# zpelgrims/pota

Hardware: AMD Instinct MI355X
Metric: bidir redistribution Msamples/s at 4K, double-gauss 50mm (higher is better)
Workload: dtype f64

## Files before the change

pota_amd/csrc/lentil_hip.hip:

```cpp
#include <hip/hip_runtime.h>
#include <hip/hip_ext.h>

#include <algorithm>
#include <atomic>
#include <chrono>
#include <cmath>
#include <cstdio>
#include <cstdlib>
#include <cstring>
#include <deque>
#include <mutex>
#include <new>
#include <string>
#include <vector>

#include "lentil_kernels.h"
#include "lentil_closest_replay.h"
#include "lentil_tl_chroma_mgpu.h"
#include "lentil_lens_jit.h"
#include "lentil_camera_rays.h"
#include "lentil_trace_points.h"
#include "lentil_list_draws.h"
#include "generated/embedded_sources.inc"

// ... 191 lines not shown
  uint32_t last_scan_launches = 0;
  int32_t dirty_lo = 0, dirty_hi = 0;
  bool dirty_known = false;
  hipEvent_t scans_done = nullptr;
  uint32_t margin_low_rate = 10;
  uint32_t batch_margin16 = 4;
  uint32_t unknown_credit = 7;
  hipEvent_t ev_solve = nullptr, ev_slow1 = nullptr;
  hipStream_t aux_stream = nullptr;
  hipEvent_t ev_crypto = nullptr;
  bool crypto_direct_enqueued = false;
  bool streams_concurrent = false;
  hipStream_t slow1_stream = nullptr;
  hipEvent_t ev_slow = nullptr, ev_round = nullptr;
  bool early_resolve_pending = false;
  bool late_resolve_done = false;
  bool resolved_valid = false;
  hipEvent_t ev_acc1 = nullptr, ev_res = nullptr;
  hipStream_t pub_stream = nullptr;
  hipEvent_t pub_done = nullptr;
  bool pass_pending = false;
  bool closest_deferred = false;
  uint32_t visit_id_base = 0;
  DevCounters *d_ctr = nullptr;
  std::vector<DevCounters> h_ctr;
  DevCounters *h_ctr_pinned = nullptr;
  bool h_ctr_valid = false;
  lentil_draw_record *d_log = nullptr;
  uint64_t log_cap = 0;
  bool timed_draw = false, timed_resolve = false;
  hipEvent_t ev_scan_k[2] = {nullptr, nullptr};
  bool scan_kernel_timed = false;
  uint32_t xor_state[4] = {123456789u, 362436069u, 521288629u, 88675123u};
  uint32_t *d_xor = nullptr, *d_tlc_res = nullptr;
  uint64_t *d_tlc_off = nullptr;
  uint2 *d_tlc_tasks = nullptr;
  uint64_t tlc_res_cap = 0, tlc_off_cap = 0, tlc_tasks_cap = 0;
  uint4 *d_xor_jump = nullptr, *d_tlc_entry = nullptr;
  uint64_t *d_tlc_val = nullptr;
  uint64_t tlc_entry_cap = 0, tlc_val_cap = 0;
  std::vector<uint32_t> tlc_gids;
  bool tlc_have_entries = false, tlc_rewalk = false;
  uint32_t *d_tlc_bound = nullptr, *d_tlc_probed = nullptr, *d_tlc_occ = nullptr;
  uint64_t tlc_bound_cap = 0, tlc_probed_cap = 0, tlc_occ_cap = 0, tlc_occ_n = 0, tlc_occ_slots = 0;
  bool tlc_occ_valid = false, pass_rerun = false;
  uint64_t tlc_items = 0, tlc_dependent = 0, tlc_gathered = 0;
  double lens_housing_radius = 0.0;
  float4 *d_dummy = nullptr;
  float *d_cam_keys = nullptr;
  float shutter_t0 = 0.0f, shutter_inv_dt = 1.0f;
  uint32_t n_cam_keys = 0;
  bool async_end = true;
  bool clear_pending = false;
  hipEvent_t ev_pre_clear = nullptr, ev_clear = nullptr;
  int ready_blocks = 2;
  struct Slot {
    hipEvent_t ev[5] = {nullptr, nullptr, nullptr, nullptr, nullptr};
    hipEvent_t ev_scan_k[2] = {nullptr, nullptr};
    hipEvent_t ev_tail = nullptr;
    DevCounters *h_ctr_pinned = nullptr;
    bool timing_open = false;
    bool timed_draw = false, timed_resolve = false, scan_kernel_timed = false;
  } slots[3];
  int slot = 0;
  struct Inflight {
    int slot = 0;
    bool abandoned = false;
    bool resolve_requested = false;
    StreamTail t;
    VisitsDev V{};
    bool have_visits = false;
  };
  std::deque<Inflight> inflight;
  bool holds_turn = false;
  lentil_pass_totals totals{};
  std::vector<std::string> notes;
  lentil_probe_fn probe_fn = nullptr;
  void *probe_user = nullptr;
  bool probe_c2w_given = false;
  float probe_c2w[16];
  std::vector<float> h_cam_keys;
  float *d_c2w_keys = nullptr;
  bool c2w_keys_valid = false;
// ... 48 lines not shown
static std::mutex g_stall_notes_mutex;
static std::vector<std::string> g_stall_notes;

static int fail(lentil_hip_ctx *ctx, int code, const std::string &msg) {
  if (ctx) ctx->err = msg; else g_err = msg;
  return code;
}
#define HIP_TRY(ctx, call)                                                                   \
  do {                                                                                       \
    hipError_t e_ = (call);                                                                  \
    if (e_ != hipSuccess)                                                                    \
      return fail(ctx, LENTIL_ERR_HIP, std::string(#call) + ": " + hipGetErrorString(e_));   \
  } while (0)
static int settle(lentil_hip_ctx *ctx);
static int probe_round(lentil_hip_ctx *ctx, int ci, const DrawArgs &da, hipStream_t st);
static int join_clear(lentil_hip_ctx *ctx);
static void harvest_ready(lentil_hip_ctx *ctx);
static int resolve_range(lentil_hip_ctx *ctx, uint64_t p_begin, uint64_t p_end);
#define CHECK_CTX_PIPELINED(ctx) \
  if (!(ctx)) return fail(nullptr, LENTIL_ERR_INVALID, "null context")
#define CHECK_CTX(ctx)                                                     \
  do {                                                                     \
    if (!(ctx)) return fail(nullptr, LENTIL_ERR_INVALID, "null context"); \
    if (!(ctx)->inflight.empty()) {                                        \
      const int rc_settle_ = settle(ctx);                                  \
      if (rc_settle_) return rc_settle_;                                   \
    }                                                                      \
    if ((ctx)->clear_pending) {                                            \
      const int rc_join_ = join_clear(ctx);                                \
      if (rc_join_) return rc_join_;                                       \
    }                                                                      \
  } while (0)

static int join_clear(lentil_hip_ctx *ctx) {
  if (!ctx->clear_pending) return LENTIL_OK;
  HIP_TRY(ctx, hipSetDevice(ctx->device));
  HIP_TRY(ctx, hipStreamWaitEvent(ctx->stream, ctx->ev_clear, 0));
  ctx->clear_pending = false;
  return LENTIL_OK;
}

static inline void ht_mark(lentil_hip_ctx *ctx, const char *what) {
  if (!host_trace_passes()) return;
  if (ctx->trace.passes_left < 0) ctx->trace.passes_left = host_trace_passes();
  if (ctx->trace.passes_left == 0) return;
  ctx->trace.marks.emplace_back(what, (int64_t)std::chrono::duration_cast<std::chrono::nanoseconds>(
// ... 84 lines not shown
  return LENTIL_OK;
}

LENTIL_API int lentil_hip_create(int device, lentil_hip_ctx **out_ctx) {
  if (!out_ctx) return fail(nullptr, LENTIL_ERR_INVALID, "out_ctx is null");
  *out_ctx = nullptr;
  int count = 0;
  hipError_t e = hipGetDeviceCount(&count);
  if (e != hipSuccess || count <= 0)
    return fail(nullptr, LENTIL_ERR_HIP, std::string("no HIP device: ") + hipGetErrorString(e));
  if (device < 0 || device >= count) return fail(nullptr, LENTIL_ERR_INVALID, "device index out of range");
  lentil_hip_ctx *ctx = new (std::nothrow) lentil_hip_ctx();
  if (!ctx) return fail(nullptr, LENTIL_ERR_NOMEM, "out of host memory");
  ctx->device = device;
  HIP_TRY(ctx, hipSetDevice(device));
  hipDeviceProp_t prop;
  HIP_TRY(ctx, hipGetDeviceProperties(&prop, device));
  ctx->num_cu = prop.multiProcessorCount > 0 ? prop.multiProcessorCount : 256;
  HIP_TRY(ctx, hipStreamCreateWithFlags(&ctx->stream, hipStreamNonBlocking));
  for (auto &ev : ctx->ev) HIP_TRY(ctx, hipEventCreate(&ev));
  if (const char *nc = getenv("LENTIL_CHUNKS")) { ctx->n_chunks = atoi(nc); }
  if (ctx->n_chunks < 1) ctx->n_chunks = 1;
  if (ctx->n_chunks > 16) ctx->n_chunks = 16;
  HIP_TRY(ctx, hipMalloc(&ctx->d_ctr, sizeof(DevCounters) * (ctx->n_chunks + 1)));
  HIP_TRY(ctx, hipHostMalloc((void **)&ctx->h_ctr_pinned, sizeof(DevCounters) * ctx->n_chunks, hipHostMallocDefault));
  memset(ctx->h_ctr_pinned, 0, sizeof(DevCounters) * ctx->n_chunks);
  if (const char *e = getenv("LENTIL_ASYNC_END")) ctx->async_end = e[0] != '0';
  HIP_TRY(ctx, hipEventCreateWithFlags(&ctx->ev_pre_clear, hipEventDisableTiming));
  HIP_TRY(ctx, hipEventCreateWithFlags(&ctx->ev_clear, hipEventDisableTiming));
  if (const char *e = getenv("LENTIL_READY_ACCEPT_BLOCKS")) { ctx->ready_blocks = atoi(e); if (ctx->ready_blocks < 1) ctx->ready_blocks = 1; if (ctx->ready_blocks > 6) ctx->ready_blocks = 6; }
  HIP_TRY(ctx, hipEventCreate(&ctx->ev_scan_k[0]));
  HIP_TRY(ctx, hipEventCreate(&ctx->ev_scan_k[1]));
  for (int si = 0; si < 3; ++si) {
    lentil_hip_ctx::Slot &sl = ctx->slots[si];
    if (si == 0) {
      for (int i = 0; i < 5; ++i) sl.ev[i] = ctx->ev[i];
      sl.ev_scan_k[0] = ctx->ev_scan_k[0]; sl.ev_scan_k[1] = ctx->ev_scan_k[1];
      sl.h_ctr_pinned = ctx->h_ctr_pinned;
    } else {
      for (int i = 0; i < 5; ++i) HIP_TRY(ctx, hipEventCreate(&sl.ev[i]));
      HIP_TRY(ctx, hipEventCreate(&sl.ev_scan_k[0]));
      HIP_TRY(ctx, hipEventCreate(&sl.ev_scan_k[1]));
      HIP_TRY(ctx, hipHostMalloc((void **)&sl.h_ctr_pinned, sizeof(DevCounters) * ctx->n_chunks, hipHostMallocDefault));
      memset(sl.h_ctr_pinned, 0, sizeof(DevCounters) * ctx->n_chunks);
    }
    HIP_TRY(ctx, hipEventCreateWithFlags(&sl.ev_tail, hipEventDisableTiming));
  }
  HIP_TRY(ctx, hipMalloc(&ctx->d_dummy, 64 * sizeof(float4)));
  HIP_TRY(ctx, hipMemsetAsync(ctx->d_ctr, 0, sizeof(DevCounters) * (ctx->n_chunks + 1), ctx->stream));
  ctx->chunks.resize(ctx->n_chunks);
  for (auto &ch : ctx->chunks) {
    HIP_TRY(ctx, hipStreamCreateWithFlags(&ch.stream, hipStreamNonBlocking));
    HIP_TRY(ctx, hipEventCreateWithFlags(&ch.scanned, hipEventDisableTiming));
    HIP_TRY(ctx, hipEventCreateWithFlags(&ch.done, hipEventDisableTiming));
  }
  HIP_TRY(ctx, hipEventCreateWithFlags(&ctx->scans_done, hipEventDisableTiming));
  HIP_TRY(ctx, hipStreamCreateWithFlags(&ctx->pub_stream, hipStreamNonBlocking));
  HIP_TRY(ctx, hipEventCreateWithFlags(&ctx->ev_slow, hipEventDisableTiming));
  HIP_TRY(ctx, hipEventCreateWithFlags(&ctx->ev_round, hipEventDisableTiming));
  HIP_TRY(ctx, hipEventCreateWithFlags(&ctx->pub_done, hipEventDisableTiming));
  HIP_TRY(ctx, hipEventCreateWithFlags(&ctx->ev_acc1, hipEventDisableTiming));
  HIP_TRY(ctx, hipEventCreateWithFlags(&ctx->ev_res, hipEventDisableTiming));
  HIP_TRY(ctx, hipEventCreateWithFlags(&ctx->ev_solve, hipEventDisableTiming));
  HIP_TRY(ctx, hipEventCreateWithFlags(&ctx->ev_slow1, hipEventDisableTiming));
  HIP_TRY(ctx, hipStreamCreateWithFlags(&ctx->slow1_stream, hipStreamNonBlocking));
  HIP_TRY(ctx, hipEventCreateWithFlags(&ctx->ev_crypto, hipEventDisableTiming));
  { const int rc = pick_concurrent_streams(ctx); if (rc) return rc; }
  if (const char *e = getenv("LENTIL_INJECT_STALL")) ctx->inject_stall_at = atoi(e);
  if (const char *e = getenv("LENTIL_PROBE_DEVICE_CAP")) { const long long v = atoll(e); ctx->probe_dev_cap = v > 0 ? (uint64_t)v : 0; }
  if (const char *ft = getenv("LENTIL_FORCE_TABLES")) ctx->use_generated = !(ft[0] == '1');
  if (const char *fc = getenv("LENTIL_FIRST_CHUNK_FRAC")) {
    const double f = atof(fc);
// ... 132 lines not shown
    if (ch.stream) (void)hipStreamDestroy(ch.stream);
  }
  if (ctx->scans_done) (void)hipEventDestroy(ctx->scans_done);
  if (ctx->pub_stream) { (void)hipStreamSynchronize(ctx->pub_stream); (void)hipStreamDestroy(ctx->pub_stream); }
  if (ctx->pub_done) (void)hipEventDestroy(ctx->pub_done);
  if (ctx->ev_slow) (void)hipEventDestroy(ctx->ev_slow);
  if (ctx->ev_round) (void)hipEventDestroy(ctx->ev_round);
  if (ctx->ev_pre_clear) (void)hipEventDestroy(ctx->ev_pre_clear);
  if (ctx->ev_clear) (void)hipEventDestroy(ctx->ev_clear);
  for (lentil_hip_ctx::Slot &sl : ctx->slots) {
    for (hipEvent_t e : sl.ev) if (e) (void)hipEventDestroy(e);
    if (sl.ev_scan_k[0]) (void)hipEventDestroy(sl.ev_scan_k[0]);
    if (sl.ev_scan_k[1]) (void)hipEventDestroy(sl.ev_scan_k[1]);
    if (sl.ev_tail) (void)hipEventDestroy(sl.ev_tail);
    if (sl.h_ctr_pinned) (void)hipHostFree(sl.h_ctr_pinned);
  }
  if (ctx->ev_acc1) (void)hipEventDestroy(ctx->ev_acc1);
  if (ctx->ev_res) (void)hipEventDestroy(ctx->ev_res);
  if (ctx->ev_solve) (void)hipEventDestroy(ctx->ev_solve);
  if (ctx->ev_slow1) (void)hipEventDestroy(ctx->ev_slow1);
  if (ctx->slow1_stream) { (void)hipStreamSynchronize(ctx->slow1_stream); (void)hipStreamDestroy(ctx->slow1_stream); }
  if (ctx->aux_stream) { (void)hipStreamSynchronize(ctx->aux_stream); (void)hipStreamDestroy(ctx->aux_stream); }
  if (ctx->ev_crypto) (void)hipEventDestroy(ctx->ev_crypto);
  (void)hipFree(ctx->d_ctr);
  (void)hipFree(ctx->d_ranges);
  (void)hipFree(ctx->d_c2w_keys);
  probe_buf_free(ctx->tlc_pb);
  probe_buf_free(ctx->ld_pb);
  for (auto &ch : ctx->chunks) probe_buf_free(ch.pb);
  if (ctx->jit_module) (void)hipModuleUnload(ctx->jit_module);
  (void)hipFree(ctx->d_bm_land); (void)hipFree(ctx->d_bm_box); (void)hipFree(ctx->d_bm_npass);
  (void)hipFree(ctx->d_xor); (void)hipFree(ctx->d_tlc_res); (void)hipFree(ctx->d_tlc_off); (void)hipFree(ctx->d_tlc_tasks);
  (void)hipFree(ctx->d_xor_jump); (void)hipFree(ctx->d_tlc_entry); (void)hipFree(ctx->d_tlc_val);
  (void)hipFree(ctx->d_tlc_bound); (void)hipFree(ctx->d_tlc_probed); (void)hipFree(ctx->d_tlc_occ);
  (void)hipFree(ctx->d_log);
  if (ctx->stream) (void)hipStreamDestroy(ctx->stream);
  delete ctx;
  return LENTIL_OK;
}

LENTIL_API const char *lentil_hip_last_error(const lentil_hip_ctx *ctx) {
  return ctx ? ctx->err.c_str() : g_err.c_str();
}

LENTIL_API const char *lentil_hip_last_redo_note(const lentil_hip_ctx *ctx) {
  return ctx ? ctx->redo_note.c_str() : "";
}
// ... 803 lines not shown
  apply_camera_motion(ctx);
  ctx->V.id_base = ctx->visit_id_base;
  rc = ensure_worklist(ctx, v->n);
  if (rc) return rc;
  ctx->have_visits = true;
  ++ctx->visits_gen;
  return LENTIL_OK;
}

LENTIL_API int lentil_hip_clear_frame(lentil_hip_ctx *ctx) {
  CHECK_CTX_PIPELINED(ctx);
  if (!ctx->inflight.empty()) { ctx->inflight.back().abandoned = true; harvest_ready(ctx); }
  if (!ctx->trace.marks.empty()) { ht_mark(ctx, "next_clear"); ht_dump(ctx); }
  ht_mark(ctx, "clear{");
  ctx->resolved_valid = false;
  if (!ctx->have_frame) return fail(ctx, LENTIL_ERR_INVALID, "no frame allocated");
  HIP_TRY(ctx, hipSetDevice(ctx->device));
  if (ctx->F.touched) {
    const uint64_t n_groups = (ctx->F.np + 63) / 64;
    uint64_t blocks = (n_groups + 255) / 256;
    const uint64_t max_blocks = (uint64_t)ctx->num_cu * 4;
    if (blocks > max_blocks) blocks = max_blocks;
    hipStream_t cs = ctx->stream;
    const bool off = ctx->streams_concurrent && ctx->stream_mode && !ctx->chunks.empty() && ctx->chunks[0].stream && !ctx->clear_pending;
    if (off) {
      cs = ctx->chunks[0].stream;
      HIP_TRY(ctx, hipEventRecord(ctx->ev_pre_clear, ctx->stream));
      HIP_TRY(ctx, hipStreamWaitEvent(cs, ctx->ev_pre_clear, 0));
    }
    hipLaunchKernelGGL(clear_touched_kernel, dim3((unsigned)blocks), dim3(256), 0, cs, ctx->F, n_groups);
    HIP_TRY(ctx, hipGetLastError());
    if (off) {
      HIP_TRY(ctx, hipEventRecord(ctx->ev_clear, cs));
      ctx->clear_pending = true;
    }
    ctx->F.touched = nullptr;
    ctx->F.touched_px = nullptr;
  } else {
  { const int rcj = join_clear(ctx); if (rcj) return rcj; }
  uint64_t p0 = 0, p1 = ctx->F.np;
  if (ctx->dirty_known && !ctx->pass_pending) {
    p0 = (uint64_t)(ctx->dirty_lo < 0 ? 0 : ctx->dirty_lo) * ctx->P.xres;
    p1 = (uint64_t)(ctx->dirty_hi < ctx->dirty_lo ? ctx->dirty_lo : ctx->dirty_hi) * ctx->P.xres;
    if (p1 > ctx->F.np) p1 = ctx->F.np;
    if (p0 > p1) p0 = p1;
  }
  if (p1 > p0) {
    HIP_TRY(ctx, hipMemsetAsync(ctx->F.acc + p0 * ctx->F.stride, 0, (p1 - p0) * ctx->F.stride * sizeof(float), ctx->stream));
    if (ctx->F.zkey) HIP_TRY(ctx, hipMemsetAsync(ctx->F.zkey + p0, 0xFF, (p1 - p0) * sizeof(unsigned long long), ctx->stream));
    if (ctx->F.zkey_dbg) HIP_TRY(ctx, hipMemsetAsync(ctx->F.zkey_dbg + p0, 0xFF, (p1 - p0) * sizeof(unsigned long long), ctx->stream));
  }
  }
  { const int rc = crypto_clear(ctx); if (rc) return rc; }
  ctx->F.dir = nullptr;
  ctx->cleared_since_pass = true;
  ctx->dirty_lo = ctx->dirty_hi = 0;
  ctx->dirty_known = true;
  ctx->pass_pending = false;
  ht_mark(ctx, "}clear");
  return LENTIL_OK;
}

template <typename T>
static int grow(lentil_hip_ctx *ctx, T **p, uint64_t need) {
  (void)hipFree(*p);
  *p = nullptr;
  HIP_TRY(ctx, hipMalloc((void **)p, need * sizeof(T)));
  return LENTIL_OK;
}

template <bool kStream>
static void launch_solve_po(lentil_hip_ctx *ctx, const DrawArgs &da, hipStream_t st, unsigned blocks) {
  const bool chroma = da.n_channels == 3;
  bool launched = false;
#define LENTIL_LAUNCH_GEN(NAME)                                                                          \
// ... 873 lines not shown
    }
  T.scan_launches += ctx->last_scan_launches ? ctx->last_scan_launches : 1u;
  if ((uint64_t)ctx->last_rounds > T.rounds_max) T.rounds_max = (uint64_t)ctx->last_rounds;
}

static int harvest_front(lentil_hip_ctx *ctx) {
  lentil_hip_ctx::Inflight in = ctx->inflight.front();
  ctx->inflight.pop_front();
  lentil_hip_ctx::Slot &sl = ctx->slots[in.slot];
  int rc = LENTIL_OK;
  HIP_TRY(ctx, hipSetDevice(ctx->device));
  {
    const hipError_t e = hipEventSynchronize(sl.ev[2]);
    if (e != hipSuccess) { release_turn(ctx); return fail(ctx, LENTIL_ERR_HIP, std::string("waiting for a pass's end: ") + hipGetErrorString(e)); }
  }
  {
    float ms = 0.f;
    if (hipEventElapsedTime(&ms, sl.ev[0], sl.ev[2]) == hipSuccess) {
      const double m = (double)ms + 0.3;
      if (!in.t.calibrates_now && m > ctx->longest_pass_ms && m < 200.0) { ctx->longest_pass_ms = m; ctx->longest_pass_visits = in.V.n; ctx->longest_pass_sum = ctx->est_sum_total; }
    } else (void)hipGetLastError();
  }
  const bool can_fix = !in.abandoned;
  ctx->last_blind = 1; ctx->last_fallback = 0; ctx->last_rounds = 0; ctx->last_scan_launches = 1; ctx->last_streamed = 1;
  ctx->h_ctr_valid = false;
  std::swap(ctx->V, in.V);
  std::swap(ctx->have_visits, in.have_visits);
  bool streamed = true;
  ctx->stall_redo = false;
  rc = streamed_finish(ctx, in.t, sl.h_ctr_pinned, can_fix, &streamed);
  if (rc == LENTIL_OK && can_fix) {
    if (ctx->stall_redo) rc = redo_after_stall(ctx);
    if (rc == LENTIL_OK && in.t.did_more) {
      ctx->resolved_valid = false;
      ctx->early_resolve_pending = false;
      (void)hipEventRecord(sl.ev[2], ctx->stream);
    }
    if (rc == LENTIL_OK) rc = pass_finish(ctx);
    if (rc == LENTIL_OK && in.resolve_requested && !ctx->resolved_valid) rc = resolve_range(ctx, 0, ctx->F.np);
  }
  ctx->stall_redo = false;
  ++ctx->totals.deferred;
  if (in.abandoned) ++ctx->totals.abandoned;
  if (rc == LENTIL_OK) account_pass(ctx);
  std::swap(ctx->V, in.V);
  std::swap(ctx->have_visits, in.have_visits);
// ... 14 lines not shown
static void harvest_ready(lentil_hip_ctx *ctx) {
  while (!ctx->inflight.empty() && ctx->inflight.front().abandoned) {
    if (hipEventQuery(ctx->slots[ctx->inflight.front().slot].ev[2]) != hipSuccess) { (void)hipGetLastError(); return; }
    (void)harvest_front(ctx);
  }
}

static int begin_slot(lentil_hip_ctx *ctx) {
  lentil_hip_ctx::Slot &cur = ctx->slots[ctx->slot];
  cur.timed_draw = ctx->timed_draw; cur.timed_resolve = ctx->timed_resolve; cur.scan_kernel_timed = ctx->scan_kernel_timed;
  const int next = (ctx->slot + 1) % 3;
  while (ctx->inflight.size() >= 2 || (!ctx->inflight.empty() && ctx->inflight.front().slot == next)) {
    const int rc = harvest_front(ctx);
    if (rc) return rc;
  }
  flush_timing(ctx, ctx->slot, false);
  ctx->slot = -1;
  flush_timing(ctx, next, true);
  ctx->slot = next;
  lentil_hip_ctx::Slot &n = ctx->slots[next];
  for (int i = 0; i < 5; ++i) ctx->ev[i] = n.ev[i];
  ctx->ev_scan_k[0] = n.ev_scan_k[0]; ctx->ev_scan_k[1] = n.ev_scan_k[1];
  ctx->h_ctr_pinned = n.h_ctr_pinned;
  ctx->timed_draw = ctx->timed_resolve = false; ctx->scan_kernel_timed = false;
  n.timing_open = true;
  return LENTIL_OK;
}

LENTIL_API int lentil_hip_set_async(lentil_hip_ctx *ctx, int on) {
  CHECK_CTX(ctx);
  ctx->async_end = on != 0;
  return LENTIL_OK;
}

LENTIL_API int lentil_hip_pass_totals(lentil_hip_ctx *ctx, lentil_pass_totals *out, int reset) {
  CHECK_CTX(ctx);
  if (!out) return fail(ctx, LENTIL_ERR_INVALID, "out is null");
  HIP_TRY(ctx, hipSetDevice(ctx->device));
  for (int si = 0; si < 3; ++si) flush_timing(ctx, si, true);
  ctx->slots[ctx->slot].timing_open = false;
  *out = ctx->totals;
  if (reset) { ctx->totals = lentil_pass_totals{}; ctx->notes.clear(); }
  return LENTIL_OK;
}

static int redistribute_impl(lentil_hip_ctx *ctx) {
// ... 29 lines not shown
  const lentil_params &P = ctx->P;
  if (P.cameraType == LENTIL_POLYNOMIAL_OPTICS && !ctx->have_lens)
    return fail(ctx, LENTIL_ERR_INVALID, "polynomial optics needs set_lens");
  if (P.bokeh_enable_image && !ctx->have_bokeh) return fail(ctx, LENTIL_ERR_INVALID, "bokeh_enable_image needs set_bokeh");
  if (ctx->V.n_extra + 1 != ctx->F.n_aovs)
    return fail(ctx, LENTIL_ERR_INVALID, "visit stream carries a different number of AOVs than the frame");
  for (uint32_t k = 1; k < ctx->F.n_aovs; ++k)
    if (ctx->V.n && !ctx->V.extra[k - 1] && !(ctx->F.debug_mask & (1u << k)))
      return fail(ctx, LENTIL_ERR_INVALID, "an extra AOV column is null");
  if (probing(ctx) && P.cameraType == LENTIL_POLYNOMIAL_OPTICS && P.abb_chromatic != 0.0f)
    return fail(ctx, LENTIL_ERR_UNSUPPORTED, "occlusion probes with polynomial optics and abb_chromatic != 0 (three wavelengths per attempt, "
                                             "src/lentil_filter.cpp:248-299): not built; the thin lens is probed with any abb_chromatic");
  if (ctx->F.debug_mask && ctx->closest_deferred && !ctx->comm)
    return fail(ctx, LENTIL_ERR_UNSUPPORTED, "the lentil_debug AOV is exchanged between GPUs by lentil_hip_allreduce / _exchange_bands only");
  HIP_TRY(ctx, hipSetDevice(ctx->device));
  { const int rc = crypto_before_pass(ctx); if (rc) return rc; }
  if (ctx->crypto_direct_enqueued) {
    HIP_TRY(ctx, hipStreamWaitEvent(ctx->stream, ctx->ev_crypto, 0));
    ctx->crypto_direct_enqueued = false;
  }
  ctx->resolved_valid = false;
  ctx->early_resolve_pending = false;
  ctx->late_resolve_done = false;
  const int C = ctx->n_chunks;
  if (ctx->pass_pending) ctx->dirty_known = false;
  ctx->pass_pending = true;
  { const int rc = begin_slot(ctx); if (rc) return rc; }
  HIP_TRY(ctx, hipMemsetAsync(ctx->d_ctr, 0, sizeof(DevCounters) * (C + 1), ctx->stream));
  HIP_TRY(ctx, hipEventRecord(ctx->ev[0], ctx->stream));
  ctx->last_rounds = 0;
  ctx->scan_kernel_timed = false;
  ctx->h_ctr_valid = false;
  ctx->last_blind = ctx->last_fallback = 0;
  ctx->last_streamed = 0;
  for (auto &ch : ctx->chunks) { ch.heavy_pending = false; ch.probe_counted = false; }
  ctx->last_scan_launches = 0;
  bool streamed = false, deferred = false;
  const bool tl_chroma = P.cameraType == LENTIL_THINLENS && P.abb_chromatic > 0.0f;
  if (tl_chroma) {
    { const int rc = join_clear(ctx); if (rc) return rc; }
    { const int rc = redistribute_tl_chroma(ctx); if (rc) return rc; }
    streamed = true;
  } else {
    const int rc = redistribute_streamed(ctx, &streamed, &deferred);
    if (rc) return rc;
    if (ctx->stall_redo) return LENTIL_OK;
  }
  if (!streamed) { const int rc = join_clear(ctx); if (rc) return rc; }
  if (!streamed && ctx->V.n) {
    ScanPlan plan;
    {
      const int rc = plan_scan(ctx, plan);
      if (rc) return rc;
    }
    const uint32_t M = plan.M;
    for (int ci = 0; ci < C; ++ci) {
      lentil_hip_ctx::Chunk &ch = ctx->chunks[ci];
      if (M) {
        auto bound = [&](int i) -> uint64_t {
          if (i <= 0) return 0;
          if (i >= C) return plan.n_tiles;
          const double f0 = C > 1 ? ctx->first_chunk_frac : 1.0;
          const double x = f0 + (1.0 - f0) * (double)(i - 1) / (double)(C - 1);
          const uint64_t b = (uint64_t)((double)plan.n_tiles * x);
          return b > plan.n_tiles ? plan.n_tiles : b;
        };
        ch.tile_begin = bound(ci);
        ch.tile_end = bound(ci + 1);
        ch.v_begin = ch.tile_begin * plan.sa.ppt * M;
        ch.v_end = ch.tile_end * plan.sa.ppt * M;
        if (ch.v_begin > ctx->V.n) ch.v_begin = ctx->V.n;
// ... 109 lines not shown
      int rounds = 0;
      bool all = true;
      for (const auto &ch : ctx->chunks) {
        all = all && ch.have_est;
        items += ch.est_items; sum += ch.est_sum;
        if (ch.est_rounds > rounds) rounds = ch.est_rounds;
      }
      if (all) { ctx->have_total_est = true; ctx->est_items_total = items; ctx->est_sum_total = sum; ctx->est_rounds_total = rounds; }
    }
  }
  if (ctx->F.zkey_dbg && ctx->V.n && !ctx->closest_deferred) {
    hipLaunchKernelGGL(debug_gather_kernel, dim3((unsigned)ctx->num_cu * 8), dim3(256), 0, ctx->stream, ctx->F, ctx->V, P,
                       ctx->have_lens ? ctx->hlens.length : 0.0);
    HIP_TRY(ctx, hipGetLastError());
  }
  if (ctx->F.zkey && ctx->V.n && !ctx->closest_deferred) {
    hipLaunchKernelGGL(closest_gather_kernel, dim3((unsigned)ctx->num_cu * 8), dim3(256), 0, ctx->stream, ctx->F, ctx->V);
    HIP_TRY(ctx, hipGetLastError());
  }
  if (ctx->early_resolve_pending) {
    ctx->early_resolve_pending = false;
    if (ctx->F.dir && ctx->F.touched && !ctx->last_fallback) {
      if (!ctx->late_resolve_done) {
        HIP_TRY(ctx, hipStreamWaitEvent(ctx->stream, ctx->ev_res, 0));
        const int rc = launch_resolve_half(ctx, ctx->stream, 2u);
        if (rc) return rc;
      }
      ctx->resolved_valid = true;
    } else {
      HIP_TRY(ctx, hipStreamWaitEvent(ctx->stream, ctx->ev_res, 0));
    }
  }
  HIP_TRY(ctx, hipEventRecord(ctx->ev[2], ctx->stream));
  ctx->timed_draw = true;
  if (deferred) return LENTIL_OK;
  return pass_finish(ctx);
}

static int pass_finish(lentil_hip_ctx *ctx) {
  const int C = ctx->n_chunks;
  if (ctx->V.n) {
    if (!ctx->h_ctr_valid) {
      HIP_TRY(ctx, hipMemcpyAsync(ctx->h_ctr_pinned, ctx->d_ctr, sizeof(DevCounters) * C, hipMemcpyDeviceToHost, ctx->stream));
      HIP_TRY(ctx, hipStreamSynchronize(ctx->stream));
      ctx->h_ctr.assign(ctx->h_ctr_pinned, ctx->h_ctr_pinned + C);
      ctx->h_ctr_valid = true;
    }
    if (ctx->probe_dev_fn) {
      for (size_t ci = 0; ci < ctx->h_ctr.size(); ++ci) {
        const DevCounters &k = ctx->h_ctr[ci];
        ctx->n_probes += k.probe_n; ctx->n_probes_occluded += k.probe_occ; ctx->n_dev_overflows += k.probe_over;
        if (k.probe_max > ctx->dev_longest) ctx->dev_longest = k.probe_max;
        if (k.fallback & 64ull) { probe_abandon(ctx); return fail(ctx, LENTIL_ERR_NOMEM, "occlusion probes: a list of " + std::to_string(k.probe_max) + " segments did not fit its buffers: the frame is incomplete"); }
      }
    }
    unsigned long long dropped = 0;
// ... 65 lines not shown
    const uint64_t chunks = ((ctx->F.np + 63) / 64 + 63) / 64;
    uint64_t blocks = chunks;
    const uint64_t max_blocks = (uint64_t)ctx->num_cu * 8;
    if (blocks > max_blocks) blocks = max_blocks;
    hipLaunchKernelGGL(resolve_touched_kernel, dim3((unsigned)blocks), dim3(256), lds, st, ctx->F, ctx->d_resolved, only_touched);
  } else {
    int per_cu = 4;
    if (const char *e = getenv("LENTIL_EARLY_RESOLVE_BLOCKS")) { per_cu = atoi(e); if (per_cu < 1) per_cu = 1; if (per_cu > 8) per_cu = 8; }
    uint64_t blocks = (ctx->F.np + 255) / 256;
    const uint64_t max_blocks = (uint64_t)ctx->num_cu * (uint64_t)per_cu;
    if (blocks > max_blocks) blocks = max_blocks;
    hipLaunchKernelGGL(resolve_kernel, dim3((unsigned)blocks), dim3(256), lds, st, ctx->F, ctx->d_resolved, (uint64_t)0, ctx->F.np);
  }
  HIP_TRY(ctx, hipGetLastError());
  return LENTIL_OK;
}

LENTIL_API int lentil_hip_resolve(lentil_hip_ctx *ctx) {
  CHECK_CTX_PIPELINED(ctx);
  if (!ctx->have_frame) return fail(ctx, LENTIL_ERR_INVALID, "no frame allocated");
  if (!ctx->inflight.empty() && !ctx->inflight.back().abandoned) ctx->inflight.back().resolve_requested = true;
  { const int rcj = join_clear(ctx); if (rcj) return rcj; }
  ht_mark(ctx, "resolve");
  if (ctx->resolved_valid) {
    HIP_TRY(ctx, hipSetDevice(ctx->device));
    HIP_TRY(ctx, hipEventRecord(ctx->ev[3], ctx->stream));
    HIP_TRY(ctx, hipEventRecord(ctx->ev[4], ctx->stream));
    ctx->timed_resolve = true;
    return LENTIL_OK;
  }
  return resolve_range(ctx, 0, ctx->F.np);
}

static int check_rows(lentil_hip_ctx *ctx, uint32_t row_begin, uint32_t n_rows) {
  if (!ctx->have_frame) return fail(ctx, LENTIL_ERR_INVALID, "no frame allocated");
  if ((uint64_t)row_begin + n_rows > (uint64_t)ctx->P.yres) return fail(ctx, LENTIL_ERR_INVALID, "row range exceeds the frame");
  return LENTIL_OK;
}

LENTIL_API int lentil_hip_resolve_rows(lentil_hip_ctx *ctx, uint32_t row_begin, uint32_t n_rows) {
  CHECK_CTX(ctx);
  const int rc = check_rows(ctx, row_begin, n_rows);
  if (rc) return rc;
  return resolve_range(ctx, (uint64_t)row_begin * ctx->P.xres, (uint64_t)(row_begin + n_rows) * ctx->P.xres);
}

LENTIL_API int lentil_hip_pack_rows(lentil_hip_ctx *ctx, uint32_t row_begin, uint32_t n_rows, void *dev_dst) {
  CHECK_CTX(ctx);
  int rc = check_rows(ctx, row_begin, n_rows);
  if (rc) return rc;
  if (!n_rows) return LENTIL_OK;
  if (!dev_dst) return fail(ctx, LENTIL_ERR_INVALID, "dev_dst is null");
  HIP_TRY(ctx, hipSetDevice(ctx->device));
// ... 1112 lines not shown
```

pota_amd/csrc/lentil_stream_pass.h:

```cpp
#pragma once


static int streamed_finish(lentil_hip_ctx *ctx, StreamTail &t, const DevCounters *pinned, bool can_fix, bool *streamed) {
  const int C = ctx->n_chunks;
  lentil_hip_ctx::Chunk &ch = ctx->chunks[0];
  int rc;
  ctx->h_ctr.assign(pinned, pinned + C);
  ctx->h_ctr_valid = true;
  ctx->last_streamed = 1;
  const DevCounters c = ctx->h_ctr[0];
  ch.was_blind = true;
  if (c.probe_snap[0]) {
    char buf[640];
    int n = snprintf(buf, sizeof buf, "[probe] epoch %u: accept blocks begun %u of %u when the last item was done; per XCD begun:", ctx->epoch, c.probe_snap[33], c.probe_snap[34]);
    for (int x = 0; x < 8; ++x) n += snprintf(buf + n, sizeof buf - n, " %u", c.probe_snap[1 + x]);
    const char *kinds[3] = {"second round's solve waves resident", "second round's straggler waves resident", "first round's straggler waves resident"};
    for (int k = 0; k < 3; ++k) {
      n += snprintf(buf + n, sizeof buf - n, " | %s:", kinds[k]);
      for (int x = 0; x < 8; ++x) n += snprintf(buf + n, sizeof buf - n, " %u", c.probe_snap[9 + 8 * k + x]);
    }
    fprintf(stderr, "%s\n", buf);
  }
  if (c.fallback || c.stuck) {
    char note[768];
// ... 386 lines not shown
  return d1;
}
static DrawArgs stream_end_args(const DrawArgs &base, const StreamForm &f) {
  DrawArgs d = stream_round_args(base, f, f.blind_rounds >= 2 ? f.blind_rounds - 1 : 0);
  d.slow_indirect = 0; d.slow_cap = f.slow_cap_all;
  d.slow_live = 0;
  return d;
}
static DrawArgs stream_gated_accept_args(const DrawArgs &base, const StreamForm &f) {
  DrawArgs d2 = stream_end_args(base, f);
  d2.lean_gate = 1;
  return d2;
}

static int stream_enqueue_head(lentil_hip_ctx *ctx, const StreamForm &f, const ScanPlan &plan, const PublishArgs &pa, const DrawArgs &base) {
  lentil_hip_ctx::Chunk &ch = ctx->chunks[0];
  int rc;
  HIP_TRY(ctx, hipEventRecord(ctx->ev[0], ctx->stream));
  if ((rc = launch_scan(ctx, plan, ch, ctx->d_ctr, true))) return rc;
  ctx->last_scan_launches = 1;
  HIP_TRY(ctx, hipEventRecord(ch.scanned, ctx->stream));
  HIP_TRY(ctx, hipEventRecord(ctx->ev[1], ctx->stream));
  HIP_TRY(ctx, hipEventRecord(ctx->scans_done, ctx->stream));
  if (ctx->crypto && ctx->aux_stream && f.crypto_overlap) {
    HIP_TRY(ctx, hipStreamWaitEvent(ctx->aux_stream, ctx->scans_done, 0));
    if ((rc = crypto_enqueue_direct(ctx, ctx->aux_stream))) return rc;
    HIP_TRY(ctx, hipEventRecord(ctx->ev_crypto, ctx->aux_stream));
    ctx->crypto_direct_enqueued = true;
  }
  HIP_TRY(ctx, hipStreamWaitEvent(ctx->pub_stream, ctx->ev[0], 0));
  hipLaunchKernelGGL(publish_kernel, dim3((unsigned)ctx->publish_waves), dim3(64), 0, ctx->pub_stream, pa);
  HIP_TRY(ctx, hipGetLastError());
  HIP_TRY(ctx, hipEventRecord(ctx->pub_done, ctx->pub_stream));
  if (f.live) {
    hipLaunchKernelGGL(solve_slow_kernel, dim3(base.slow_waves), dim3(64), coop_lds_bytes(ctx->hlens.n_terms), ctx->pub_stream, base);
    HIP_TRY(ctx, hipGetLastError());
    HIP_TRY(ctx, hipEventRecord(ctx->ev_slow, ctx->pub_stream));
  }
  HIP_TRY(ctx, hipStreamWaitEvent(ch.stream, ctx->ev[0], 0));
  launch_solve_po<true>(ctx, base, ch.stream, f.a_blocks);
  HIP_TRY(ctx, hipGetLastError());
  HIP_TRY(ctx, hipEventRecord(ch.done, ch.stream));
  return LENTIL_OK;
}

static int stream_enqueue_late_resolve(lentil_hip_ctx *ctx, hipStream_t st) {
  if (!ctx->early_resolve_pending) return LENTIL_OK;
  HIP_TRY(ctx, hipStreamWaitEvent(st, ctx->ev_res, 0));
  const int rc = launch_resolve_half(ctx, st, 2u);
  if (!rc) ctx->late_resolve_done = true;
  return rc;
}

static int stream_enqueue_decoupled_accept(lentil_hip_ctx *ctx, const StreamForm &f, const DrawArgs &base) {
  lentil_hip_ctx::Chunk &ch = ctx->chunks[0];
  hipStream_t rs = ctx->chunks[1].stream;
  int rc;
  HIP_TRY(ctx, hipStreamWaitEvent(ch.stream, ctx->pub_done, 0));
  HIP_TRY(ctx, hipStreamWaitEvent(ch.stream, ctx->scans_done, 0));
  HIP_TRY(ctx, hipEventRecord(ctx->ev_round, ch.stream));
  if (f.resolve_after_scan) {
    if (ctx->clear_pending) HIP_TRY(ctx, hipStreamWaitEvent(rs, ctx->ev_clear, 0));
    HIP_TRY(ctx, hipStreamWaitEvent(rs, ctx->scans_done, 0));
    if ((rc = launch_resolve_half(ctx, rs, 0u))) return rc;
  }
  const DrawArgs d0 = stream_first_accept_args(ctx, base, f);
  if (f.ready_accept) hipLaunchKernelGGL(accept_kernel<3>, dim3(f.accept1_blocks), dim3(256), 0, ch.stream, d0);
  else hipLaunchKernelGGL(accept_kernel<1>, dim3(f.accept1_blocks), dim3(256), 0, ch.stream, d0);
  HIP_TRY(ctx, hipGetLastError());
  HIP_TRY(ctx, hipEventRecord(ctx->ev_acc1, ch.stream));
  if (f.resolves_early) {
    HIP_TRY(ctx, hipStreamWaitEvent(rs, ctx->ev_acc1, 0));
    if ((rc = launch_resolve_half(ctx, rs, f.resolve_after_scan ? 1u : 0u))) return rc;
    HIP_TRY(ctx, hipEventRecord(ctx->ev_res, rs));
    ctx->early_resolve_pending = true;
  }
  return LENTIL_OK;
}

static int stream_enqueue_lean_tail(lentil_hip_ctx *ctx, const StreamForm &f, const DrawArgs &base, hipStream_t *tail) {
  hipStream_t ls = ctx->chunks[0].stream;
  HIP_TRY(ctx, hipStreamWaitEvent(ls, ctx->ev_slow, 0));
  hipLaunchKernelGGL(reset_round_kernel, dim3(1), dim3(1), 0, ls, ctx->d_ctr, 0u, 1u);
  hipLaunchKernelGGL(accept_kernel<2>, dim3(f.accept_blocks), dim3(256), 0, ls, stream_gated_accept_args(base, f));
  HIP_TRY(ctx, hipGetLastError());
// ... 80 lines not shown
      HIP_TRY(ctx, hipEventRecord(ctx->ev_slow, ctx->pub_stream));
      HIP_TRY(ctx, hipStreamWaitEvent(ctx->stream, ctx->ev_slow, 0));
    } else {
      launch_solve(ctx, da, ctx->stream, (unsigned)ctx->num_cu);
    }
    hipLaunchKernelGGL(accept_kernel<0>, dim3(f.accept_blocks), dim3(256), 0, ctx->stream, da);
    HIP_TRY(ctx, hipGetLastError());
  }
  *tail = ctx->stream;
  return stream_enqueue_late_resolve(ctx, ctx->stream);
}

static int stream_end(lentil_hip_ctx *ctx, DeviceTurn &turn, StreamTail &t, bool *streamed, bool *deferred) {
  hipStream_t tail = t.tail;
  ht_mark(ctx, "all_launched");
  ctx->clear_pending = false;
  HIP_TRY(ctx, hipMemcpyAsync(ctx->h_ctr_pinned, ctx->d_ctr, sizeof(DevCounters) * ctx->n_chunks, hipMemcpyDeviceToHost, tail));
  const bool defer = ctx->async_end && t.lean && !ctx->crypto && !ctx->F.zkey && !ctx->F.zkey_dbg &&
                     !ctx->comm && !ctx->closest_deferred && !t.inject && !host_trace_passes() && ctx->inflight.size() < 2;
  if (defer) {
    lentil_hip_ctx::Slot &sl = ctx->slots[ctx->slot];
    HIP_TRY(ctx, hipEventRecord(sl.ev_tail, tail));
    if (tail != ctx->stream) HIP_TRY(ctx, hipStreamWaitEvent(ctx->stream, sl.ev_tail, 0));
    t.deferred = true;
    lentil_hip_ctx::Inflight in;
    in.slot = ctx->slot; in.t = t; in.V = ctx->V; in.have_visits = ctx->have_visits;
    ctx->inflight.push_back(in);
    turn.keep();
    ctx->last_streamed = 1;
    ++ctx->last_blind;
    *deferred = true;
    *streamed = true;
    return LENTIL_OK;
  }
  HIP_TRY(ctx, hipStreamSynchronize(tail));
  ht_mark(ctx, "tail_synced");
  if (tail != ctx->stream) HIP_TRY(ctx, hipStreamSynchronize(ctx->stream));
  ht_mark(ctx, "main_synced");
  const double ms = std::chrono::duration<double, std::milli>(std::chrono::steady_clock::now() - t.pass_t0).count();
  if (!t.calibrates_now && ms > ctx->longest_pass_ms && ms < 200.0) {
    ctx->longest_pass_ms = ms; ctx->longest_pass_visits = ctx->V.n; ctx->longest_pass_sum = ctx->est_sum_total;
  }
  ++ctx->last_blind;
  return streamed_finish(ctx, t, ctx->h_ctr_pinned, true, streamed);
}

// ... 33 lines not shown
```

Baseline: 42060.

## Triple-buffer device counters and trim cross-stream waits in the streamed pass

```diff
diff --git a/pota_amd/csrc/lentil_hip.hip b/pota_amd/csrc/lentil_hip.hip
--- a/pota_amd/csrc/lentil_hip.hip
+++ b/pota_amd/csrc/lentil_hip.hip
@@ -237,7 +237,7 @@
   bool pass_pending = false;
   bool closest_deferred = false;
   uint32_t visit_id_base = 0;
-  DevCounters *d_ctr = nullptr;
+  DevCounters *d_ctr = nullptr, *d_ctr_base = nullptr;
   std::vector<DevCounters> h_ctr;
   DevCounters *h_ctr_pinned = nullptr;
   bool h_ctr_valid = false;
@@ -268,12 +268,15 @@
   bool async_end = true;
   bool clear_pending = false;
   hipEvent_t ev_pre_clear = nullptr, ev_clear = nullptr;
+  hipEvent_t wipe_after = nullptr;
   int ready_blocks = 2;
   struct Slot {
     hipEvent_t ev[5] = {nullptr, nullptr, nullptr, nullptr, nullptr};
     hipEvent_t ev_scan_k[2] = {nullptr, nullptr};
     hipEvent_t ev_tail = nullptr;
     DevCounters *h_ctr_pinned = nullptr;
+    DevCounters *d_ctr = nullptr;
+    bool ctr_fresh = false;
     bool timing_open = false;
     bool timed_draw = false, timed_resolve = false, scan_kernel_timed = false;
   } slots[3];
@@ -368,6 +371,7 @@
 #define CHECK_CTX(ctx)                                                     \
   do {                                                                     \
     if (!(ctx)) return fail(nullptr, LENTIL_ERR_INVALID, "null context"); \
+    (ctx)->wipe_after = nullptr;                                           \
     if (!(ctx)->inflight.empty()) {                                        \
       const int rc_settle_ = settle(ctx);                                  \
       if (rc_settle_) return rc_settle_;                                   \
@@ -498,7 +502,9 @@
   if (const char *nc = getenv("LENTIL_CHUNKS")) { ctx->n_chunks = atoi(nc); }
   if (ctx->n_chunks < 1) ctx->n_chunks = 1;
   if (ctx->n_chunks > 16) ctx->n_chunks = 16;
-  HIP_TRY(ctx, hipMalloc(&ctx->d_ctr, sizeof(DevCounters) * (ctx->n_chunks + 1)));
+  const size_t ctr_stride = ((sizeof(DevCounters) * (size_t)(ctx->n_chunks + 1) + 4095u) / 4096u) * 4096u;
+  HIP_TRY(ctx, hipMalloc((void **)&ctx->d_ctr_base, ctr_stride * 3));
+  ctx->d_ctr = ctx->d_ctr_base;
   HIP_TRY(ctx, hipHostMalloc((void **)&ctx->h_ctr_pinned, sizeof(DevCounters) * ctx->n_chunks, hipHostMallocDefault));
   memset(ctx->h_ctr_pinned, 0, sizeof(DevCounters) * ctx->n_chunks);
   if (const char *e = getenv("LENTIL_ASYNC_END")) ctx->async_end = e[0] != '0';
@@ -521,9 +527,10 @@
       memset(sl.h_ctr_pinned, 0, sizeof(DevCounters) * ctx->n_chunks);
     }
     HIP_TRY(ctx, hipEventCreateWithFlags(&sl.ev_tail, hipEventDisableTiming));
+    sl.d_ctr = reinterpret_cast<DevCounters *>(reinterpret_cast<char *>(ctx->d_ctr_base) + (size_t)si * ctr_stride);
   }
   HIP_TRY(ctx, hipMalloc(&ctx->d_dummy, 64 * sizeof(float4)));
-  HIP_TRY(ctx, hipMemsetAsync(ctx->d_ctr, 0, sizeof(DevCounters) * (ctx->n_chunks + 1), ctx->stream));
+  HIP_TRY(ctx, hipMemsetAsync(ctx->d_ctr_base, 0, ctr_stride * 3, ctx->stream));
   ctx->chunks.resize(ctx->n_chunks);
   for (auto &ch : ctx->chunks) {
     HIP_TRY(ctx, hipStreamCreateWithFlags(&ch.stream, hipStreamNonBlocking));
@@ -702,7 +709,7 @@
   if (ctx->slow1_stream) { (void)hipStreamSynchronize(ctx->slow1_stream); (void)hipStreamDestroy(ctx->slow1_stream); }
   if (ctx->aux_stream) { (void)hipStreamSynchronize(ctx->aux_stream); (void)hipStreamDestroy(ctx->aux_stream); }
   if (ctx->ev_crypto) (void)hipEventDestroy(ctx->ev_crypto);
-  (void)hipFree(ctx->d_ctr);
+  (void)hipFree(ctx->d_ctr_base);
   (void)hipFree(ctx->d_ranges);
   (void)hipFree(ctx->d_c2w_keys);
   probe_buf_free(ctx->tlc_pb);
@@ -1552,11 +1559,15 @@
     const uint64_t max_blocks = (uint64_t)ctx->num_cu * 4;
     if (blocks > max_blocks) blocks = max_blocks;
     hipStream_t cs = ctx->stream;
-    const bool off = ctx->streams_concurrent && ctx->stream_mode && !ctx->chunks.empty() && ctx->chunks[0].stream && !ctx->clear_pending;
+    const bool off = ctx->streams_concurrent && ctx->stream_mode && ctx->chunks.size() >= 2 && ctx->chunks[1].stream && !ctx->clear_pending;
     if (off) {
-      cs = ctx->chunks[0].stream;
-      HIP_TRY(ctx, hipEventRecord(ctx->ev_pre_clear, ctx->stream));
-      HIP_TRY(ctx, hipStreamWaitEvent(cs, ctx->ev_pre_clear, 0));
+      cs = ctx->chunks[1].stream;
+      if (ctx->wipe_after) {
+        HIP_TRY(ctx, hipStreamWaitEvent(cs, ctx->wipe_after, 0));
+      } else {
+        HIP_TRY(ctx, hipEventRecord(ctx->ev_pre_clear, ctx->stream));
+        HIP_TRY(ctx, hipStreamWaitEvent(cs, ctx->ev_pre_clear, 0));
+      }
     }
     hipLaunchKernelGGL(clear_touched_kernel, dim3((unsigned)blocks), dim3(256), 0, cs, ctx->F, n_groups);
     HIP_TRY(ctx, hipGetLastError());
@@ -1581,6 +1592,7 @@
     if (ctx->F.zkey_dbg) HIP_TRY(ctx, hipMemsetAsync(ctx->F.zkey_dbg + p0, 0xFF, (p1 - p0) * sizeof(unsigned long long), ctx->stream));
   }
   }
+  ctx->wipe_after = nullptr;
   { const int rc = crypto_clear(ctx); if (rc) return rc; }
   ctx->F.dir = nullptr;
   ctx->cleared_since_pass = true;
@@ -2500,6 +2512,7 @@
     } else (void)hipGetLastError();
   }
   const bool can_fix = !in.abandoned;
+  if (can_fix) ctx->wipe_after = nullptr;
   ctx->last_blind = 1; ctx->last_fallback = 0; ctx->last_rounds = 0; ctx->last_scan_launches = 1; ctx->last_streamed = 1;
   ctx->h_ctr_valid = false;
   std::swap(ctx->V, in.V);
@@ -2560,6 +2573,7 @@
   for (int i = 0; i < 5; ++i) ctx->ev[i] = n.ev[i];
   ctx->ev_scan_k[0] = n.ev_scan_k[0]; ctx->ev_scan_k[1] = n.ev_scan_k[1];
   ctx->h_ctr_pinned = n.h_ctr_pinned;
+  ctx->d_ctr = n.d_ctr;
   ctx->timed_draw = ctx->timed_resolve = false; ctx->scan_kernel_timed = false;
   n.timing_open = true;
   return LENTIL_OK;
@@ -2635,12 +2649,13 @@
   ctx->resolved_valid = false;
   ctx->early_resolve_pending = false;
   ctx->late_resolve_done = false;
+  ctx->wipe_after = nullptr;
   const int C = ctx->n_chunks;
   if (ctx->pass_pending) ctx->dirty_known = false;
   ctx->pass_pending = true;
   { const int rc = begin_slot(ctx); if (rc) return rc; }
-  HIP_TRY(ctx, hipMemsetAsync(ctx->d_ctr, 0, sizeof(DevCounters) * (C + 1), ctx->stream));
-  HIP_TRY(ctx, hipEventRecord(ctx->ev[0], ctx->stream));
+  if (!ctx->slots[ctx->slot].ctr_fresh) HIP_TRY(ctx, hipMemsetAsync(ctx->d_ctr, 0, sizeof(DevCounters) * (C + 1), ctx->stream));
+  ctx->slots[ctx->slot].ctr_fresh = false;
   ctx->last_rounds = 0;
   ctx->scan_kernel_timed = false;
   ctx->h_ctr_valid = false;
@@ -2651,6 +2666,7 @@
   bool streamed = false, deferred = false;
   const bool tl_chroma = P.cameraType == LENTIL_THINLENS && P.abb_chromatic > 0.0f;
   if (tl_chroma) {
+    HIP_TRY(ctx, hipEventRecord(ctx->ev[0], ctx->stream));
     { const int rc = join_clear(ctx); if (rc) return rc; }
     { const int rc = redistribute_tl_chroma(ctx); if (rc) return rc; }
     streamed = true;
@@ -2659,7 +2675,11 @@
     if (rc) return rc;
     if (ctx->stall_redo) return LENTIL_OK;
   }
-  if (!streamed) { const int rc = join_clear(ctx); if (rc) return rc; }
+  if (!streamed) {
+    HIP_TRY(ctx, hipEventRecord(ctx->ev[0], ctx->stream));
+    const int rc = join_clear(ctx);
+    if (rc) return rc;
+  }
   if (!streamed && ctx->V.n) {
     ScanPlan plan;
     {
@@ -2815,6 +2835,7 @@
     ctx->early_resolve_pending = false;
     if (ctx->F.dir && ctx->F.touched && !ctx->last_fallback) {
       if (!ctx->late_resolve_done) {
+        ctx->wipe_after = nullptr;
         HIP_TRY(ctx, hipStreamWaitEvent(ctx->stream, ctx->ev_res, 0));
         const int rc = launch_resolve_half(ctx, ctx->stream, 2u);
         if (rc) return rc;
@@ -2824,7 +2845,7 @@
       HIP_TRY(ctx, hipStreamWaitEvent(ctx->stream, ctx->ev_res, 0));
     }
   }
-  HIP_TRY(ctx, hipEventRecord(ctx->ev[2], ctx->stream));
+  if (!(deferred && ctx->wipe_after)) HIP_TRY(ctx, hipEventRecord(ctx->ev[2], ctx->stream));
   ctx->timed_draw = true;
   if (deferred) return LENTIL_OK;
   return pass_finish(ctx);
@@ -2936,13 +2957,8 @@
   if (!ctx->inflight.empty() && !ctx->inflight.back().abandoned) ctx->inflight.back().resolve_requested = true;
   { const int rcj = join_clear(ctx); if (rcj) return rcj; }
   ht_mark(ctx, "resolve");
-  if (ctx->resolved_valid) {
-    HIP_TRY(ctx, hipSetDevice(ctx->device));
-    HIP_TRY(ctx, hipEventRecord(ctx->ev[3], ctx->stream));
-    HIP_TRY(ctx, hipEventRecord(ctx->ev[4], ctx->stream));
-    ctx->timed_resolve = true;
-    return LENTIL_OK;
-  }
+  if (ctx->resolved_valid) return LENTIL_OK;
+  ctx->wipe_after = nullptr;
   return resolve_range(ctx, 0, ctx->F.np);
 }
 
diff --git a/pota_amd/csrc/lentil_stream_pass.h b/pota_amd/csrc/lentil_stream_pass.h
--- a/pota_amd/csrc/lentil_stream_pass.h
+++ b/pota_amd/csrc/lentil_stream_pass.h
@@ -432,6 +432,11 @@
   HIP_TRY(ctx, hipEventRecord(ch.scanned, ctx->stream));
   HIP_TRY(ctx, hipEventRecord(ctx->ev[1], ctx->stream));
   HIP_TRY(ctx, hipEventRecord(ctx->scans_done, ctx->stream));
+  {
+    lentil_hip_ctx::Slot &nx = ctx->slots[(ctx->slot + 1) % 3];
+    HIP_TRY(ctx, hipMemsetAsync(nx.d_ctr, 0, sizeof(DevCounters) * (ctx->n_chunks + 1), ctx->stream));
+    nx.ctr_fresh = true;
+  }
   if (ctx->crypto && ctx->aux_stream && f.crypto_overlap) {
     HIP_TRY(ctx, hipStreamWaitEvent(ctx->aux_stream, ctx->scans_done, 0));
     if ((rc = crypto_enqueue_direct(ctx, ctx->aux_stream))) return rc;
@@ -441,6 +446,7 @@
   HIP_TRY(ctx, hipStreamWaitEvent(ctx->pub_stream, ctx->ev[0], 0));
   hipLaunchKernelGGL(publish_kernel, dim3((unsigned)ctx->publish_waves), dim3(64), 0, ctx->pub_stream, pa);
   HIP_TRY(ctx, hipGetLastError());
+  HIP_TRY(ctx, hipStreamWaitEvent(ctx->pub_stream, ctx->scans_done, 0));
   HIP_TRY(ctx, hipEventRecord(ctx->pub_done, ctx->pub_stream));
   if (f.live) {
     hipLaunchKernelGGL(solve_slow_kernel, dim3(base.slow_waves), dim3(64), coop_lds_bytes(ctx->hlens.n_terms), ctx->pub_stream, base);
@@ -448,9 +454,10 @@
     HIP_TRY(ctx, hipEventRecord(ctx->ev_slow, ctx->pub_stream));
   }
   HIP_TRY(ctx, hipStreamWaitEvent(ch.stream, ctx->ev[0], 0));
+  if (ctx->clear_pending) HIP_TRY(ctx, hipStreamWaitEvent(ch.stream, ctx->ev_clear, 0));
   launch_solve_po<true>(ctx, base, ch.stream, f.a_blocks);
   HIP_TRY(ctx, hipGetLastError());
-  HIP_TRY(ctx, hipEventRecord(ch.done, ch.stream));
+  if (!f.decoupled) HIP_TRY(ctx, hipEventRecord(ch.done, ch.stream));
   return LENTIL_OK;
 }
 
@@ -467,10 +474,8 @@
   hipStream_t rs = ctx->chunks[1].stream;
   int rc;
   HIP_TRY(ctx, hipStreamWaitEvent(ch.stream, ctx->pub_done, 0));
-  HIP_TRY(ctx, hipStreamWaitEvent(ch.stream, ctx->scans_done, 0));
-  HIP_TRY(ctx, hipEventRecord(ctx->ev_round, ch.stream));
+  if (!f.lean_pass) HIP_TRY(ctx, hipEventRecord(ctx->ev_round, ch.stream));
   if (f.resolve_after_scan) {
-    if (ctx->clear_pending) HIP_TRY(ctx, hipStreamWaitEvent(rs, ctx->ev_clear, 0));
     HIP_TRY(ctx, hipStreamWaitEvent(rs, ctx->scans_done, 0));
     if ((rc = launch_resolve_half(ctx, rs, 0u))) return rc;
   }
@@ -597,6 +602,8 @@
     lentil_hip_ctx::Slot &sl = ctx->slots[ctx->slot];
     HIP_TRY(ctx, hipEventRecord(sl.ev_tail, tail));
     if (tail != ctx->stream) HIP_TRY(ctx, hipStreamWaitEvent(ctx->stream, sl.ev_tail, 0));
+    ctx->wipe_after = sl.ev_tail;
+    HIP_TRY(ctx, hipEventRecord(ctx->ev[2], tail));
     t.deferred = true;
     lentil_hip_ctx::Inflight in;
     in.slot = ctx->slot; in.t = t; in.V = ctx->V; in.have_visits = ctx->have_visits;
```

Result: no change. 42500, median of 6 (+1.0%).
